# malaire/reed-solomon-16

Measured on AMD Instinct MI355X. Metric: encode+decode GiB/s (device-resident, 1024B shards); % of HBM roofline, higher is better.
Workload: dtype u16; 1 GPU; 32768:32768 x 1024 B encode + 100%-loss decode per GPU (BASELINE configs[3]); original_count=32768, recovery_count=32768, parallelism=independent stripes x 1 (weak, no collective), column_slices=1, decode_issue=serial: rs16_decode_device after the encode

## Files before the change

include/rs16.h:

```cpp
#ifndef RS16_H
#define RS16_H

#include <stddef.h>
#include <stdint.h>

#ifdef __cplusplus
extern "C" {
#endif

typedef enum rs16_error_code {
    RS16_OK = 0,
    RS16_DIFFERENT_SHARD_SIZE = 1,
    RS16_DUPLICATE_ORIGINAL_SHARD_INDEX = 2,
    RS16_DUPLICATE_RECOVERY_SHARD_INDEX = 3,
    RS16_INVALID_ORIGINAL_SHARD_INDEX = 4,
    RS16_INVALID_RECOVERY_SHARD_INDEX = 5,
    RS16_INVALID_SHARD_SIZE = 6,
    RS16_NOT_ENOUGH_SHARDS = 7,
    RS16_TOO_FEW_ORIGINAL_SHARDS = 8,
    RS16_TOO_MANY_ORIGINAL_SHARDS = 9,
    RS16_UNSUPPORTED_SHARD_COUNT = 10,
    RS16_DEVICE_ERROR = 100,
    RS16_INVALID_ARGUMENT = 101
} rs16_error_code;
// ... 174 lines not shown
int rs16_engine_set_stamps(rs16_engine* eng, void* d_buf, int prog, rs16_error* err);
const char* rs16_prog_name(int prog);

enum {
    RS16_DIAG_FORCE_VOFF64 = 1,
    RS16_DIAG_EVAL_TWO_KERNEL = 2,
    RS16_DIAG_EVAL_FULL = 4,
    RS16_DIAG_NO_COLUMN = 8,
    RS16_DIAG_FORCE_COLUMN = 16,
    RS16_DIAG_TILE_LAST = 32,
    RS16_DIAG_NO_TILE_LAST = 64,
    RS16_DIAG_FD_LDS = 128,
    RS16_DIAG_COL_RADIX4 = 256,
    RS16_DIAG_NO_IDENTITY = 512,
    RS16_DIAG_NO_MID_DIRECT = 1024,
    RS16_DIAG_WIDE_TWIDDLES = 2048
};
int rs16_engine_set_diagnostics(rs16_engine* eng, int flags);
int rs16_set_diagnostics(int flags);

void rs16_host_mul(const void* in, void* out, size_t bytes, uint16_t log_m);
void rs16_host_mul_narrow(const void* in, void* out, size_t bytes, uint16_t log_m);
uint32_t rs16_host_twiddle(uint32_t index, uint32_t* log_m, uint32_t* table20);
int rs16_host_twiddle_narrow(uint32_t index);
uint64_t rs16_host_fast_div_check(uint32_t divisor, uint32_t n0, uint32_t count, uint32_t step);
typedef struct rs16_pass_consts {
    uint32_t voff32, full_lanes, nslab;
    uint32_t quads, threads, load_shb, store_shb, reg_bits, row_sets;
    uint64_t rs_in, rs_seg, rs_out;
} rs16_pass_consts;
int rs16_host_pass_consts(int prog, int T, uint32_t lo, uint64_t s_in, uint64_t s_out, uint64_t s_seg, uint64_t s_rest,
                          uint32_t qrow, uint32_t chunk, uint32_t row_base_in, uint32_t in_rows_mask, int diag,
                          rs16_pass_consts* out);
int rs16_host_pass_consts_many(int prog, int T, uint32_t lo, size_t n, const uint64_t* s_in, const uint64_t* s_out,
                               const uint64_t* s_seg, const uint64_t* s_rest, const uint32_t* qrow, uint32_t chunk,
                               uint32_t row_base_in, uint32_t in_rows_mask, int diag, rs16_pass_consts* out);
int rs16_host_update_consts(uint32_t rows, uint64_t shard_bytes, uint32_t n, uint32_t* quads_per_lane,
                            uint32_t* nslab, uint32_t* rows_per_wave, uint64_t* blocks);

const char* rs16_version(void);

#ifdef __cplusplus
}
#endif
#endif
```

reed-solomon-16_amd/csrc/rs16_api.cpp:

```cpp
#include <atomic>
#include <rccl/rccl.h>

#include <algorithm>
#include <cstdio>
#include <cstring>
#include <new>
#include <vector>

#include "rs16_engine.hpp"
#include "rs16_pass_common.hpp"

using namespace rs16;

extern "C" size_t rs16_error_message(const rs16_error* e, char* buf, size_t len) {
    char tmp[256];
    unsigned long long a = e->v0, b = e->v1, c = e->v2;
    switch (e->code) {
    case RS16_OK: snprintf(tmp, sizeof tmp, "ok"); break;
    case RS16_DIFFERENT_SHARD_SIZE:
        snprintf(tmp, sizeof tmp, "different shard size: expected %llu bytes, got %llu bytes", a, b);
        break;
    case RS16_DUPLICATE_ORIGINAL_SHARD_INDEX: snprintf(tmp, sizeof tmp, "duplicate original shard index: %llu", a); break;
    case RS16_DUPLICATE_RECOVERY_SHARD_INDEX: snprintf(tmp, sizeof tmp, "duplicate recovery shard index: %llu", a); break;
    case RS16_INVALID_ORIGINAL_SHARD_INDEX:
// ... 68 lines not shown
    const HostTables& t = host_tables();
    if (index >= GF_MODULUS) return ~0u;
    if (log_m) *log_m = t.skew[index];
    if (table20) memcpy(table20, &t.skew_tab[(size_t)index * TAB_DWORDS], 20 * sizeof(uint32_t));
    return t.skew[index] == GF_MODULUS ? 0u : t.exp[t.skew[index]];
}
extern "C" int rs16_host_twiddle_narrow(uint32_t index) { return twiddle_narrow(index) ? 1 : 0; }
extern "C" uint64_t rs16_host_fast_div_check(uint32_t divisor, uint32_t n0, uint32_t count, uint32_t step) {
    const FastDiv f = fast_div_of(divisor);
    uint64_t bad = 0;
    for (uint64_t i = 0, n = n0; i < count && n < ((uint64_t)1 << 32); i++, n += step)
        bad += fast_div((uint32_t)n, f.mul, f.one) != (uint32_t)n / divisor;
    return bad;
}

extern "C" int rs16_host_pass_consts_many(int prog, int T, uint32_t lo, size_t n, const uint64_t* s_in,
                                          const uint64_t* s_out, const uint64_t* s_seg, const uint64_t* s_rest,
                                          const uint32_t* qrow, uint32_t chunk, uint32_t row_base_in,
                                          uint32_t in_rows_mask, int diag, rs16_pass_consts* out) {
    if (prog < 0 || prog >= NUM_PROGS || T < 0 || T > 8 || !out) return 0;
    const PassKernel& k = pass_kernel_of(prog, T);
    if (!k.fn) return 0;
    PassArgs a{};
    a.lo = lo, a.chunk = chunk, a.row_base_in = row_base_in, a.in_rows_mask = in_rows_mask;
    a.diag = (uint32_t)diag;
    for (size_t i = 0; i < n; i++) {
        a.S_in = s_in[i], a.S_out = s_out[i], a.S_seg = s_seg[i], a.S_rest = s_rest[i], a.qrow = qrow[i];
        const PassConsts c = pass_launch_consts(k, T, a);
        rs16_pass_consts& o = out[i];
        o.voff32 = c.voff32, o.full_lanes = c.full_lanes, o.nslab = c.nslab;
        o.quads = (uint32_t)k.quads, o.threads = (uint32_t)k.threads;
        o.load_shb = (uint32_t)k.load_shb, o.store_shb = (uint32_t)k.store_shb;
        o.reg_bits = (uint32_t)k.reg_bits, o.row_sets = k.quads >= 64 ? 1u : 64u / (uint32_t)k.quads;
        o.rs_in = c.rs_in, o.rs_seg = c.rs_seg, o.rs_out = c.rs_out;
    }
    return 1;
}
extern "C" int rs16_host_pass_consts(int prog, int T, uint32_t lo, uint64_t s_in, uint64_t s_out, uint64_t s_seg,
                                     uint64_t s_rest, uint32_t qrow, uint32_t chunk, uint32_t row_base_in,
                                     uint32_t in_rows_mask, int diag, rs16_pass_consts* out) {
    return rs16_host_pass_consts_many(prog, T, lo, 1, &s_in, &s_out, &s_seg, &s_rest, &qrow, chunk, row_base_in,
                                      in_rows_mask, diag, out);
}
extern "C" int rs16_host_update_consts(uint32_t rows, uint64_t shard_bytes, uint32_t n, uint32_t* quads_per_lane,
                                       uint32_t* nslab, uint32_t* rows_per_wave, uint64_t* blocks) {
    if (shard_bytes == 0 || (shard_bytes & 63) != 0 || shard_bytes / 8 > 0xFFFFFFFFu) return 0;
    UpdateArgs a{};
    a.S = shard_bytes, a.qrow = (uint32_t)(shard_bytes / 8), a.rows = rows;
    uint64_t nb;
    if (!update_launch_consts(a, n, &nb)) return 0;
    if (quads_per_lane) *quads_per_lane = a.quads_per_lane;
// ... 47 lines not shown
        for (uint32_t i = 0; i < g.a_count; i++) a += f[i] != 0;
        for (uint32_t i = 0; i < g.b_count; i++) b += f[GF_ORDER + i] != 0;
    } else {
        const size_t chunks = ((size_t)g.n + 63) / 64;
        std::vector<uint32_t> c(2 * chunks);
        RS16_HIP(hipMemcpy(c.data(), e->ev_main.rcount.p, c.size() * 4, hipMemcpyDeviceToHost));
        for (size_t i = 0; i < chunks; i++) a += c[2 * i], b += c[2 * i + 1];
    }
    const uint64_t want_o = g.high ? g.b_recv : g.a_recv, want_r = g.high ? g.a_recv : g.b_recv;
    const uint64_t got_o = g.high ? b : a, got_r = g.high ? a : b;
    if (got_o != want_o || got_r != want_r) return set_error(err, RS16_INVALID_ARGUMENT, got_o, got_r);
    return set_error(err, RS16_OK);
}
static constexpr int DIAG_ALL = DIAG_FORCE_VOFF64 | DIAG_EVAL_TWO_KERNEL | DIAG_EVAL_FULL | DIAG_NO_COLUMN |
                                DIAG_FORCE_COLUMN | DIAG_TILE_LAST | DIAG_NO_TILE_LAST | DIAG_FD_LDS |
                                DIAG_COL_RADIX4 | DIAG_NO_IDENTITY | DIAG_NO_MID_DIRECT | DIAG_WIDE_TWIDDLES;
extern "C" int rs16_engine_set_diagnostics(rs16_engine* e, int flags) {
    const int old = e->diag;
    e->diag = flags & DIAG_ALL;
    return old;
}
static std::atomic<int> g_default_diag{0};
extern "C" int rs16_set_diagnostics(int flags) { return g_default_diag.exchange(flags & DIAG_ALL); }
extern "C" int rs16_prog_count(void) { return NUM_PROF; }
extern "C" const char* rs16_prog_name(int prog) {
    static const char* names[] = {"GEN_FFT",   "GEN_IFFT",   "ENC_FIRST",     "ENC_MID",
                                  "ENC_LAST",  "ENC_SINGLE", "DEC_FIRST",     "DEC_MID",
                                  "DEC_LAST",  "DEC_SINGLE", "DEC_HALF_LAST", "DEC_HALF_SINGLE",
                                  "DEC_HALF_FIRST", "DEC_HALF_MID", "EVAL_POLY", "COL_ENC", "COL_DEC",
                                  "DEC_MID_DIRECT", "DEC_TILE_LAST"};
    static_assert(sizeof names / sizeof names[0] == NUM_PROF, "profiling names");
// ... 1546 lines not shown
```

reed-solomon-16_amd/csrc/rs16_diag.hpp:

```cpp
#pragma once
#include <hip/hip_runtime.h>
#include <stdint.h>

#ifndef RS16_STAMPS
#define RS16_STAMPS 0
#endif

#if RS16_STAMPS
namespace rs16 {
template <class Args>
__device__ __forceinline__ void diag_stamp(const Args& a, int i) {
    if (a.stamps && threadIdx.x == 0) {
        uint64_t* p = a.stamps + blockIdx.x * 16;
        p[i] = __builtin_amdgcn_s_memtime();
        if (i == 0) {
            p[14] = __builtin_amdgcn_s_memrealtime();
            p[12] = __builtin_amdgcn_s_getreg((31 << 11) | 4);
            p[13] = __builtin_amdgcn_s_getreg((31 << 11) | 20);
        }
        if (i == 11) p[15] = __builtin_amdgcn_s_memrealtime();
    }
}
}
#define RS16_STAMP(args, i) ::rs16::diag_stamp((args), (i))
// ... 16 lines not shown
```

reed-solomon-16_amd/csrc/rs16_internal.hpp:

```cpp
#pragma once
#include <hip/hip_runtime.h>
#include <stddef.h>
#include <stdint.h>

#include <vector>

#include "rs16_gf.hpp"

namespace rs16 {

struct HostTables {
    std::vector<uint16_t> exp, log, skew, log_walsh;
    std::vector<uint32_t> skew_entry;
    std::vector<uint32_t> mul_tab;
    std::vector<uint32_t> skew_tab;
    std::vector<uint32_t> col_img;
    std::vector<uint32_t> col_v;
    std::vector<uint32_t> col_k;
};
std::vector<uint32_t> mid_matrix_entries(const HostTables& t, int L);

constexpr uint32_t COL_LMIN = 6, COL_LMAX = 10;
constexpr uint32_t COL_LGEN = 11;
constexpr uint32_t COL_LCHUNK = 8;
// ... 155 lines not shown
hipError_t launch_col_multi(const ColArgs& a, bool high, hipStream_t s);

enum DiagFlags : int {
    DIAG_FORCE_VOFF64 = 1,
    DIAG_EVAL_TWO_KERNEL = 2,
    DIAG_EVAL_FULL = 4,
    DIAG_NO_COLUMN = 8,
    DIAG_FORCE_COLUMN = 16,
    DIAG_TILE_LAST = 32,
    DIAG_NO_TILE_LAST = 64,
    DIAG_FD_LDS = 128,
    DIAG_COL_RADIX4 = 256,
    DIAG_NO_IDENTITY = 512,
    DIAG_NO_MID_DIRECT = 1024,
    DIAG_WIDE_TWIDDLES = 2048,
};

constexpr size_t RS16_ZERO_BYTES = 65536;

hipError_t launch_pass(int prog, int T, const PassArgs& a, uint32_t num_tiles, hipStream_t s);
hipError_t launch_tile_last(const PassArgs& a, uint32_t num_tiles, hipStream_t s);
constexpr uint32_t MID_DIRECT_MAX = 4;
constexpr uint32_t TILE_LAST_MAX = 16;
hipError_t launch_mid_direct(const PassArgs& a, const uint32_t* mtab, uint32_t hi, uint32_t ns, hipStream_t s);

hipError_t launch_mul(uint8_t* x, size_t bytes, uint32_t entry, const uint32_t* mul_tab, hipStream_t s);
hipError_t launch_xor(uint8_t* x, const uint8_t* y, size_t bytes, hipStream_t s);
hipError_t launch_xor_chunks(uint8_t* w, size_t chunk_bytes, uint32_t nch, hipStream_t s);
hipError_t launch_copy_chunks(uint8_t* w, size_t chunk_bytes, uint32_t nch, hipStream_t s);
hipError_t launch_formal_derivative(uint8_t* out, const uint8_t* in, size_t shard_count, size_t S, hipStream_t s);
// ... 43 lines not shown
```

reed-solomon-16_amd/csrc/rs16_pass.hpp:

```cpp
#pragma once
#include "rs16_pass_common.hpp"
#include "rs16_fwht.hpp"
#include "rs16_diag.hpp"

namespace rs16 {

enum LoadMode { LD_PLAIN = 0, LD_GATHER_ENC, LD_GATHER_DEC, LD_DEC_LAST };
enum StoreMode { ST_PLAIN = 0, ST_RECOVERY, ST_RESTORE };

template <int P> struct ProgTraits;
#define RS16_PROG(P, LD, I, F, FF, ST)          \
    template <> struct ProgTraits<P> {         \
        static constexpr int LOAD = LD;        \
        static constexpr bool IFFT = I;        \
        static constexpr bool FD = F;          \
        static constexpr bool FFT = FF;        \
        static constexpr int STORE = ST;       \
        static constexpr bool ST_NT = !(I && FF);                                           \
    };
RS16_PROG(GEN_FFT, LD_PLAIN, false, false, true, ST_PLAIN)
RS16_PROG(GEN_IFFT, LD_PLAIN, true, false, false, ST_PLAIN)
RS16_PROG(ENC_FIRST, LD_GATHER_ENC, true, false, false, ST_PLAIN)
RS16_PROG(ENC_MID, LD_PLAIN, true, false, true, ST_PLAIN)
RS16_PROG(ENC_LAST, LD_PLAIN, false, false, true, ST_RECOVERY)
// ... 172 lines not shown
    }
    asm volatile("; full-item rows requested");
    return true;
}
enum RowsMode { ROWS_DIRECT = 0, ROWS_ZERO, ROWS_GENERAL };
template <int P, int T>
__device__ __forceinline__ uint32_t wave_rows_mode(const PassArgs& a, const Thr& c) {
    constexpr bool START_B = !ProgTraits<P>::IFFT;
    constexpr bool GATHER = ProgTraits<P>::LOAD == LD_GATHER_ENC;
    const WaveRows<T, START_B> wr(c, a);
    const bool below = !GATHER || wave_rows_end<T, START_B>(wr) <= a.a_count;
    const bool above = GATHER && wr.base >= a.a_count;
    const bool direct = (a.voff32 != 0) & (a.in_rows_mask == 0) & below;
    return direct ? ROWS_DIRECT : (above ? ROWS_ZERO : ROWS_GENERAL);
}
template <int P, int T> struct FastStore {
    static constexpr bool END_B = !ProgTraits<P>::FFT && T > 4;
    const PassArgs& a;
    const Thr& cs;
    bool on;
    uint64_t p;
    __device__ __forceinline__ FastStore(const PassArgs& a_, const Thr& cs_) : a(a_), cs(cs_), on(false), p(0) {
        if constexpr (FastRows<P, T>::STORE) {
            const WaveRows<T, END_B> wr(cs, a);
            on = a.full_lanes &&
                 (ProgTraits<P>::STORE != ST_RECOVERY || wave_rows_end<T, END_B>(wr) <= a.out_rows);
            p = (uint64_t)a.out + (uint64_t)wr.base * a.S_out;
        }
    }
    __device__ __forceinline__ void row(int m, uint32_t L, uint32_t H) const {
// ... 77 lines not shown
    }
};

template <int T> struct RevealEntry {
    const PassArgs& a;
    const Thr& c;
    const uint32_t* el;
    __device__ __forceinline__ uint32_t operator()(int k) const {
        const uint32_t r = row_rel<T>(c, a, (uint32_t)k) + a.row_base_out;
        return row_lost_original(a, r) ? GF_MODULUS - (el ? el[k] : a.elog[r]) : ZERO_ENTRY;
    }
};

struct NoFin {
    template <class X> __device__ __forceinline__ void operator()(const X&, const X&, int) const {}
};

template <int T, bool LB, int KB0, int KB1, bool FFT> struct LayerSeq {
    static constexpr int SH = LB ? Geo<T>::SHB : 0;
    static constexpr int NR = Geo<T>::NR;
    static constexpr bool DF = FFT && !LB && KB0 == 0 && KB1 == Geo<T>::R && NR >= 8;
    static constexpr int df_at(int g) {
        int skb[16] = {}, sgi[16] = {};
        int sp = 0, n = 0;
        skb[sp] = KB1 - 1, sgi[sp] = 0, sp++;
        while (sp > 0) {
            sp--;
            const int kb = skb[sp], gi = sgi[sp];
            if (n++ == g) return kb * 16 + gi;
            if (kb > 0) {
// ... 43 lines not shown
            asm volatile("" : "+v"(L[i]), "+v"(L[i + 1]), "+v"(L[i + 2]), "+v"(L[i + 3]), "+v"(H[i]), "+v"(H[i + 1]),
                         "+v"(H[i + 2]), "+v"(H[i + 3]));
    } else {
#pragma unroll
        for (int i = 0; i < NR; i++) asm volatile("" : "+v"(L[i]), "+v"(H[i]));
    }
}

enum { PR_NONE = 0, PR_OUT, PR_ZERO };
template <int NV> struct NarrowVar {
    static constexpr int NONE = 99;
    static constexpr int IFFT_FROM = NV == 0 ? NONE : (NV == 2 ? 1 : 0);
    static constexpr int FFT_FROM = NV == 0 ? NONE : (NV == 3 ? 1 : 0);
};

template <int P, int T, int NK, bool LB, int KB0, int KB1, bool FFT, bool IN_TAB2, int PRUNE, int G, class FIN = NoFin>
struct GroupLoop {
    static __device__ __forceinline__ void run(uint32_t (&L)[Geo<T>::NR], uint32_t (&H)[Geo<T>::NR], const Thr& c,
                                               const PassArgs& a, const uint4* tab1, const uint4* tab2,
                                               const uint32_t (&cur)[20], uint32_t zmask, const FIN& fin = FIN()) {
        using S = LayerSeq<T, LB, KB0, KB1, FFT>;
        constexpr int s = S::step_of(G), gi = S::index_of(G);
        constexpr int kb = S::kb_of(s);
        constexpr int rb = kb - S::SH;
        constexpr bool more = G + 1 < S::total();
        constexpr bool NARROW = kb >= NK;
        uint32_t nxt[20];
        if constexpr (more)
            load_table_lds(nxt, group_table<T, LB, KB0, KB1, FFT, G + 1, IN_TAB2>(c, tab1, tab2));
        __builtin_amdgcn_sched_barrier(0);
        bool need = true;
        if constexpr (PRUNE == PR_OUT)
            need = ((uint32_t)gi << (kb + 1)) < a.need_hi && ((uint32_t)(gi + 1) << (kb + 1)) > a.need_lo;
        if constexpr (PRUNE == PR_ZERO) {
            static_assert(LB && kb >= 4, "zero pruning works on 16-row blocks of layout B");
            constexpr int nb = 1 << (kb - 3);
            constexpr uint32_t all = (uint32_t)((1ull << nb) - 1);
            need = ((zmask >> (gi * nb)) & all) != all;
        }
        bool mul = true;
        if constexpr (LB && gi == 0 && ProgTraits<P>::IFFT && ProgTraits<P>::FFT) {
            const uint32_t idx = (c.b_high << (a.lo + T)) + (1u << (a.lo + kb)) + (FFT ? a.skew_fft : a.skew_ifft) - 1;
            mul = (idx & (idx + 1)) != 0;
        }
        if (need && mul) {
#pragma unroll
            for (int j = 0; j < (1 << rb); j++) {
                const int m = (gi << (rb + 1)) + j, m2 = m + (1 << rb);
                if (FFT) {
                    mul_xor_t<NARROW>(L[m], H[m], L[m2], H[m2], cur);
                    L[m2] ^= L[m];
                    H[m2] ^= H[m];
                } else {
                    L[m2] ^= L[m];
                    H[m2] ^= H[m];
                    mul_xor_t<NARROW>(L[m], H[m], L[m2], H[m2], cur);
                }
            }
        } else if (need) {
#pragma unroll
            for (int j = 0; j < (1 << rb); j++) {
                const int m = (gi << (rb + 1)) + j, m2 = m + (1 << rb);
                L[m2] ^= L[m];
                H[m2] ^= H[m];
            }
        }
#pragma unroll
        for (int j = 0; j < (1 << rb); j++) {
            const int m = (gi << (rb + 1)) + j, m2 = m + (1 << rb);
            asm volatile("" : "+v"(L[m]), "+v"(H[m]), "+v"(L[m2]), "+v"(H[m2]));
        }
        __builtin_amdgcn_sched_barrier(0);
        if constexpr (S::DF && kb == 0) fin(L, H, gi << 1);
        if constexpr (more)
            GroupLoop<P, T, NK, LB, KB0, KB1, FFT, IN_TAB2, PRUNE, G + 1, FIN>::run(L, H, c, a, tab1, tab2, nxt, zmask,
                                                                                     fin);
    }
};

__device__ __forceinline__ const uint4* lds_vgpr(const uint4* p) {
    uint32_t v = (uint32_t)(uintptr_t)(const __attribute__((address_space(3))) uint4*)p;
    asm volatile("" : "+v"(v));
    return (const uint4*)(const __attribute__((address_space(3))) uint4*)(uintptr_t)v;
}

template <int P, int T, int NK, bool LB, int KB0, int KB1, bool FFT, bool IN_TAB2, int PRUNE = PR_NONE,
          class FIN = NoFin>
__device__ __forceinline__ void layers(uint32_t (&L)[Geo<T>::NR], uint32_t (&H)[Geo<T>::NR], const Thr& c,
                                       const PassArgs& a, const uint4* tab1, const uint4* tab2,
                                       uint32_t zmask = 0, const FIN& fin = FIN()) {
    if constexpr (KB1 > KB0) {
        if constexpr (LB) {
            if constexpr (IN_TAB2) tab2 = lds_vgpr(tab2);
            else tab1 = lds_vgpr(tab1);
        }
        uint32_t t0[20];
        load_table_lds(t0, group_table<T, LB, KB0, KB1, FFT, 0, IN_TAB2>(c, tab1, tab2));
        GroupLoop<P, T, NK, LB, KB0, KB1, FFT, IN_TAB2, PRUNE, 0, FIN>::run(L, H, c, a, tab1, tab2, t0, zmask, fin);
    }
}

template <int T, int QL> struct Img {
    static constexpr int PLANE = (1 << T) * QL;
    static __device__ __forceinline__ uint32_t* at(uint2* lds, const Thr& c, uint32_t k) {
        return (uint32_t*)lds + k * QL + c.ql;
    }
};

template <int NQR> __device__ __forceinline__ bool my_round(const Thr& c, int r) {
    return NQR == 1 || c.round == (uint32_t)r;
}

template <int T, int QL, bool LB>
// ... 573 lines not shown
    const FastStore<P, T> fs;
    __device__ __forceinline__ void operator()(const uint32_t (&L)[Geo<T>::NR], const uint32_t (&H)[Geo<T>::NR]) const {
        if (fs.on) {
#pragma unroll
            for (int m = 0; m < Geo<T>::NR; m += 2) fs.row(m, L[m], H[m]);
            return;
        }
#pragma unroll
        for (int m = 0; m < Geo<T>::NR; m += 2) {
            if (a.voff32) store_row<P, T, true>(a, cs, L[m], H[m], m, nullptr, nullptr);
            else store_row<P, T, false>(a, cs, L[m], H[m], m, nullptr, nullptr);
        }
    }
};

template <int P, int T, int NV>
__device__ __forceinline__ void process_item(const PassArgs& a, const Thr& c, uint32_t tile, ItemRegs<P, T>& d,
                                             uint8_t* smem) {
    using PT = ProgTraits<P>;
    constexpr int NKI = NarrowVar<NV>::IFFT_FROM, NKF = NarrowVar<NV>::FFT_FROM;
    static_assert(NV == 0 || (PT::IFFT && PT::FFT && T > 4), "narrow variants: two-direction passes only");
    using SM = Smem<P, T>;
    using G = Geo<T>;
    constexpr int NR = G::NR;
    constexpr int R = G::R;
    constexpr int NQR = Rnd<P, T>::NQR;
    constexpr bool TWO = SM::TWO;
    constexpr bool ZERO_SKIP = P == DEC_MID && T > 4 && G::R == 4;
    constexpr bool EARLY = LayerSeq<T, false, 0, R, true>::DF && P != DEC_MID && PT::STORE != ST_RESTORE && PT::FFT &&
                           T > 4;
    constexpr bool EARLY_B = PT::IFFT && !PT::FFT && PT::STORE == ST_PLAIN && T > 4 && G::R == 4;
    uint2* lds = (uint2*)smem;
    const uint4* tab1 = (const uint4*)(smem + SM::TAB1_OFF);
// ... 32 lines not shown
            const uint32_t yl = L[m], yh = H[m];
            L[m] = H[m] = 0;
            mul_xor(L[m], H[m], yl, yh, tt);
        }
    }
    if constexpr (PT::LOAD == LD_DEC_LAST) {
        if (!d.ztile) tile_fd<T, NQR, START_B>(L, H, d.zl, d.zh, c, lds);
    }

    [[maybe_unused]] Stager<T, (SM::SHARED ? G::TSPLIT : 0)> s3s;
    bool in_b = START_B;
    if constexpr (PT::IFFT) {
        bool skip_a = false;
        if constexpr (ZERO_SKIP) skip_a = __all(d.zrow == (1u << NR) - 1);
        if constexpr (WaveStaged<P, T>::value) RS16_STAMP_ROWS(a, 6, L, H, 0, 1);
        if (!skip_a) layers<P, T, NKI, false, 0, R, false, false>(L, H, c, a, tab1, tab2);
        RS16_STAMP(a, 3);
        prio<1>();
        if constexpr (T > 4) {
            constexpr bool LS2 = SM::RESTAGE && !SM::SHARED;
            Stager<T, (LS2 ? G::TSPLIT : 0)> s3;
            if constexpr (LS2) s3.issue(a.skew_tab, TwiddleEntry<T>{a, c, 0, a.skew_fft});
            if constexpr (SM::SHARED) __syncthreads();
            exchange<T, NQR, false>(
                L, H, c, lds,
                [&]() {
                    if constexpr (LS2) s3.commit((uint4*)(smem + SM::TAB1_OFF));
                },
                [&]() {
                    if constexpr (SPLIT_FD) {
                        if (fd_few) {
// ... 21 lines not shown
        prio<2>();
    }
    if constexpr (PT::FD) {
        if constexpr (SPLIT_FD) {
            if (fd_few) fd_regs<T>(L, H);
            else tile_fd<T, NQR, true>(L, H, L, H, c, lds);
        } else {
            if (in_b) tile_fd<T, NQR, true>(L, H, L, H, c, lds);
            else tile_fd<T, NQR, false>(L, H, L, H, c, lds);
        }
        RS16_STAMP(a, 6);
    }
    if constexpr (PT::FFT) {
        if constexpr (T > 4) {
            if constexpr (WaveStaged<P, T>::value && !PT::IFFT) RS16_STAMP_ROWS(a, 6, L, H, 0, NR / 2);
            layers<P, T, NKF, true, R, (T > 4 ? T : R), true, TWO, (P == DEC_MID ? PR_OUT : PR_NONE)>(L, H, c, a, tab1,
                                                                                                  tab2);
            if constexpr (SPLIT_FD) {
                if (fd_few) {
#pragma unroll
                    for (int m = 0; m < NR; m++) {
#pragma unroll
                        for (int i = 0; i < FD_ND; i++)
                            if ((uint32_t)m == fd_m0 + i) L[m] ^= dl[i], H[m] ^= dh[i];
                    }
                }
            }
            RS16_STAMP(a, 7);
            prio<3>();
            RevealStage<P, (LateReveal<P, T>::value ? T : 0)> rs;
            if constexpr (LateReveal<P, T>::value) {
                const uint32_t* el = nullptr;
// ... 148 lines not shown
            lost_range(a, r0, r1);
            const bool any = r0 < r1;
            a.need_lo = max(a.need_lo, any ? r0 >> a.lo : 0u);
            a.need_hi = min(a.need_hi, any ? ((r1 - 1) >> a.lo) + 1 : 0u);
        }
    }
    RS16_STAMP(a, 1);
    prio<0>();
    st.template finish<EARLY>(a, c, smem);
    rcn.count();
    RS16_STAMP(a, 2);
    process_item<P, T, NV>(a, c, tile, cur, smem);
    rcn.store(a, c);
}

template <int P, int T, int NV = 0> PassKernel pass_entry() {
    using PT = ProgTraits<P>;
    return {pass_kernel<P, T, NV>, Smem<P, T>::BYTES, Geo<T>::THREADS, Geo<T>::Q,
            !PT::IFFT ? Geo<T>::SHB : 0, (!PT::FFT && T > 4) ? Geo<T>::SHB : 0, Geo<T>::R};
}
template <int P> PassKernel pass_row(int T) {
    static const PassKernel row[9] = {pass_entry<P, 0>(), pass_entry<P, 1>(), pass_entry<P, 2>(),
                                      pass_entry<P, 3>(), pass_entry<P, 4>(), pass_entry<P, 5>(),
                                      pass_entry<P, 6>(), pass_entry<P, 7>(), pass_entry<P, 8>()};
    return row[T];
}
template <int P, int NV> PassKernel narrow_row(int T) {
    static const PassKernel row[4] = {pass_entry<P, 5, NV>(), pass_entry<P, 6, NV>(), pass_entry<P, 7, NV>(),
                                      pass_entry<P, 8, NV>()};
    return T >= 5 ? row[T - 5] : PassKernel{};
}

}
```

reed-solomon-16_amd/csrc/rs16_pass_common.hpp:

```cpp
#pragma once
#include "rs16_internal.hpp"

namespace rs16 {

typedef void (*PassFn)(PassArgs);
struct PassKernel {
    PassFn fn;
    int lds;
    int threads;
    int quads;
    int load_shb, store_shb;
    int reg_bits;
};
struct PassConsts {
    uint32_t nslab, voff32, full_lanes;
    uint64_t rs_in, rs_seg, rs_out;
};
PassConsts pass_launch_consts(const PassKernel& k, int T, const PassArgs& a);
const PassKernel& pass_kernel_of(int prog, int T);
constexpr int NARROW_VARIANTS = 4;
PassKernel pass_kernels_enc(int prog, int T, int nv);
PassKernel pass_kernels_dec(int prog, int T, int nv);

#if defined(__HIPCC__) || defined(__HIP__)
typedef const __attribute__((address_space(4))) uint32_t* cu32p;

__device__ __forceinline__ uint32_t uni(uint32_t v) { return __builtin_amdgcn_readfirstlane(v); }

__host__ __device__ constexpr int vmcnt_wait(int n) { return (n & 15) | ((n >> 4) << 14) | (7 << 4) | (15 << 8); }

__device__ __forceinline__ void load_table_lds(uint32_t (&t)[20], const uint4* p) {
// ... 59 lines not shown
```

reed-solomon-16_amd/csrc/rs16_pass_launch.hip:

```cpp
#include <algorithm>

#include "rs16_pass_common.hpp"

namespace rs16 {

struct KernelTable {
    PassKernel k[NUM_PROGS][9][NARROW_VARIANTS];
    KernelTable() {
        for (int prog = 0; prog < NUM_PROGS; prog++)
            for (int T = 0; T <= 8; T++)
                for (int nv = 0; nv < NARROW_VARIANTS; nv++) {
                    const PassKernel e = pass_kernels_enc(prog, T, nv);
                    k[prog][T][nv] = e.fn ? e : pass_kernels_dec(prog, T, nv);
                }
    }
};
static const PassKernel& find_kernel(int prog, int T, int nv) {
    static const KernelTable table;
    return table.k[prog][T][nv];
}

static const PassKernel& pick_kernel(int prog, int T, int ni, int nf) {
    for (int nv = 1; nv < NARROW_VARIANTS; nv++) {
        const int vi = nv == 2 ? 1 : 0, vf = nv == 3 ? 1 : 0;
// ... 10 lines not shown
    PassConsts c;
    c.nslab = (a.qrow + k.quads - 1) / k.quads;
    {
        const uint64_t hws = k.quads >= 64 ? 1 : 64 / k.quads;
        const uint64_t smax = std::max(std::max(a.S_in, a.S_out), std::max(a.S_seg, a.S_rest));
        const uint64_t span = (uint64_t)1 << (T + a.lo);
        const bool fits = (hws - 1) * ((uint64_t)16 << a.lo) * smax + 8 * (uint64_t)a.qrow <= ((uint64_t)1 << 32);
        const bool aligned = a.chunk % span == 0 && a.row_base_in % span == 0;
        c.voff32 = fits && aligned && !(a.diag & DIAG_FORCE_VOFF64) ? 1u : 0u;
    }
    c.rs_in = a.S_in << (a.lo + k.load_shb);
    c.rs_seg = a.S_seg << (a.lo + k.load_shb);
    c.rs_out = a.S_out << (a.lo + k.store_shb);
    const bool full = c.voff32 && a.qrow % k.quads == 0 && a.in_rows_mask == 0 && c.rs_out < ((uint64_t)1 << 28);
    c.full_lanes = full ? 1u : 0u;
    return c;
}

hipError_t launch_pass(int prog, int T, const PassArgs& args, uint32_t num_tiles, hipStream_t s) {
    if (prog < 0 || prog >= NUM_PROGS || T < 0 || T > 8) return hipErrorInvalidValue;
    if (num_tiles == 0 || args.qrow == 0) return hipSuccess;
    PassArgs a = args;
    int ni = T, nf = T;
    if (!(a.diag & DIAG_WIDE_TWIDDLES)) {
        const uint32_t bh_max = (a.tile_base + (a.stripe_tiles ? a.stripe_tiles : num_tiles) - 1) >> a.lo;
        ni = first_narrow_layer(a.lo, T, a.skew_ifft, bh_max);
        nf = first_narrow_layer(a.lo, T, a.skew_fft, bh_max);
    }
    const PassKernel& k = pick_kernel(prog, T, ni, nf);
    const PassConsts pc = pass_launch_consts(k, T, a);
    a.nslab = pc.nslab;
    a.ntiles = num_tiles;
    const uint32_t nwg = num_tiles * a.nslab;
    if (a.need_hi == 0) a.need_hi = 1u << T;
    a.voff32 = pc.voff32;
    a.fd_lds = (a.diag & DIAG_FD_LDS) ? 1u : 0u;
    a.rs_in = pc.rs_in, a.rs_seg = pc.rs_seg, a.rs_out = pc.rs_out;
    a.full_lanes = pc.full_lanes;
    const FastDiv dn = fast_div_of(a.nslab), ds = fast_div_of(a.stripe_tiles);
    a.nslab_mul = dn.mul, a.nslab_one = dn.one;
    a.stripe_mul = ds.mul, a.stripe_one = ds.one;
    const size_t lds = (size_t)k.lds;
    if (lds > 65536) {
        hipError_t e = hipFuncSetAttribute((const void*)k.fn, hipFuncAttributeMaxDynamicSharedMemorySize, (int)lds);
        if (e != hipSuccess) return e;
    }
    dim3 grid(nwg), block(k.threads);
    hipLaunchKernelGGL(k.fn, grid, block, lds, s, a);
    return hipGetLastError();
}

}
```

reed-solomon-16_amd/rs16/__init__.py:

```python
from __future__ import annotations

import atexit
import ctypes as C
import weakref
from typing import Iterable, Iterator, Optional, Tuple

import numpy as np

from ._lib import RS16Error, lib

__all__ = [
    "Error", "Engine", "default_engine", "ReedSolomonEncoder", "ReedSolomonDecoder", "RateEncoder",
    "RateDecoder", "EncoderResult", "DecoderResult", "encode", "decode", "encode_device", "decode_device",
    "supports", "validate", "use_high_rate", "encode_device_batch", "decode_device_batch", "encoder_work_count", "decoder_work_count",
    "RATE_DEFAULT", "RATE_HIGH", "RATE_LOW", "GF_ORDER", "GF_MODULUS", "set_diagnostics",
    "DIAG_FORCE_VOFF64", "DIAG_EVAL_TWO_KERNEL", "DIAG_EVAL_FULL", "DIAG_NO_COLUMN", "DIAG_FORCE_COLUMN",
    "DIAG_TILE_LAST", "DIAG_NO_TILE_LAST", "DIAG_FD_LDS", "DIAG_COL_RADIX4", "DIAG_NO_IDENTITY", "DIAG_NO_MID_DIRECT", "DIAG_WIDE_TWIDDLES", "encode_host", "decode_host",
    "encode_host_batch", "decode_host_batch", "decode_prepare", "decode_device_prepared",
    "UpdatePlan", "update_recovery_device", "UPDATE_MAX_SHARDS",
    "encode_host_multi", "decode_host_multi", "Comm", "column_slice", "scatter_columns", "gather_columns",
]

GF_ORDER = 65536
GF_MODULUS = 65535
DIAG_FORCE_VOFF64, DIAG_EVAL_TWO_KERNEL, DIAG_EVAL_FULL, DIAG_NO_COLUMN, DIAG_FORCE_COLUMN = 1, 2, 4, 8, 16
DIAG_TILE_LAST, DIAG_NO_TILE_LAST, DIAG_FD_LDS, DIAG_COL_RADIX4, DIAG_NO_IDENTITY = 32, 64, 128, 256, 512
DIAG_NO_MID_DIRECT = 1024
DIAG_WIDE_TWIDDLES = 2048
_diag_default = 0


def set_diagnostics(flags: int, engine: Optional["Engine"] = None) -> int:
    global _diag_default
    if engine is not None:
        return engine.set_diagnostics(flags)
    old, _diag_default = _diag_default, flags
    for e in list(_live_engines):
        if getattr(e, "h", None):
            e.set_diagnostics(flags)
    return old
RATE_DEFAULT, RATE_HIGH, RATE_LOW = 0, 1, 2
_RATES = {"default": 0, "high": 1, "low": 2, 0: 0, 1: 1, 2: 2}

# ... 797 lines not shown
```

reed-solomon-16_amd/rs16/_lib.py:

```python
from __future__ import annotations

import ctypes as C
import os
from pathlib import Path

PKG_ROOT = Path(__file__).resolve().parents[1]
LIB_PATH = Path(os.environ.get("RS16_LIB", PKG_ROOT / "build" / "librs16.so"))


class RS16Error(C.Structure):
    _fields_ = [("code", C.c_int32), ("v0", C.c_uint64), ("v1", C.c_uint64), ("v2", C.c_uint64)]


class PassConsts(C.Structure):
    _fields_ = [(n, C.c_uint32) for n in ("voff32", "full_lanes", "nslab", "quads", "threads", "load_shb",
                                          "store_shb", "reg_bits", "row_sets")] + \
               [(n, C.c_uint64) for n in ("rs_in", "rs_seg", "rs_out")]


_sz, _p, _i, _e = C.c_size_t, C.c_void_p, C.c_int, C.POINTER(RS16Error)
_u32, _u64 = C.c_uint32, C.c_uint64

SIGNATURES = {
    "rs16_error_message": (_sz, [_e, C.c_char_p, _sz]),
    "rs16_version": (C.c_char_p, []),
    "rs16_host_mul": (None, [_p, _p, _sz, C.c_uint16]),
    "rs16_host_mul_narrow": (None, [_p, _p, _sz, C.c_uint16]),
    "rs16_host_twiddle": (C.c_uint32, [C.c_uint32, C.POINTER(C.c_uint32), C.POINTER(C.c_uint32)]),
    "rs16_host_twiddle_narrow": (C.c_int, [C.c_uint32]),
    "rs16_host_fast_div_check": (C.c_uint64, [C.c_uint32, C.c_uint32, C.c_uint32, C.c_uint32]),
    "rs16_host_pass_consts": (_i, [_i, _i, _u32, _u64, _u64, _u64, _u64, _u32, _u32, _u32, _u32, _i,
                                   C.POINTER(PassConsts)]),
    "rs16_host_pass_consts_many": (_i, [_i, _i, _u32, _sz, _p, _p, _p, _p, _p, _u32, _u32, _u32, _i, _p]),
    "rs16_host_update_consts": (_i, [_u32, _u64, _u32, C.POINTER(_u32), C.POINTER(_u32), C.POINTER(_u32),
                                     C.POINTER(_u64)]),
    "rs16_engine_set_profiling": (_i, [_p, _i, _e]),
    "rs16_engine_profile_read": (_i, [_p, _i, C.POINTER(C.c_double), C.POINTER(C.c_uint64), _e]),
    "rs16_engine_profile_reset": (None, [_p]),
    "rs16_prog_count": (_i, []),
    "rs16_engine_set_diagnostics": (_i, [_p, _i]),
    "rs16_prog_name": (C.c_char_p, [_i]),
    "rs16_engine_set_stamps": (_i, [_p, _p, _i, _e]),
    "rs16_engine_set_slices": (_i, [_p, _i, _e]),
    "rs16_engine_new": (_p, [_i, _e]),
    "rs16_engine_new_ex": (_p, [_i, _i, _e]),
    "rs16_set_diagnostics": (_i, [_i]),
    "rs16_engine_free": (None, [_p]),
# ... 111 lines not shown
```

Baseline: 1012 GiB/s.

## Stream late row pairs into registers during first butterfly layer in wave-staged passes

Adds a variant pass kernel for wave-staged programs that loads only the first D row pairs up front and fetches the remaining pairs from global memory inside the first layer of the IFFT/FFT butterfly loop, interleaved with compute. The aim is to overlap global-load latency with the GF multiply-xor work instead of waiting for all rows before computing. The host selects this kernel when strides fit in 32-bit offsets, no row mask is set and gather row counts align, with a diagnostic flag to disable it. The cost is extra scheduling barriers and register pressure, and the zero-skip shortcut is bypassed on this path.

```diff
diff --git a/include/rs16.h b/include/rs16.h
--- a/include/rs16.h
+++ b/include/rs16.h
@@ -212,7 +212,8 @@
     RS16_DIAG_COL_RADIX4 = 256,
     RS16_DIAG_NO_IDENTITY = 512,
     RS16_DIAG_NO_MID_DIRECT = 1024,
-    RS16_DIAG_WIDE_TWIDDLES = 2048
+    RS16_DIAG_WIDE_TWIDDLES = 2048,
+    RS16_DIAG_NO_LATE_ROWS = 4096
 };
 int rs16_engine_set_diagnostics(rs16_engine* eng, int flags);
 int rs16_set_diagnostics(int flags);
@@ -226,6 +227,7 @@
     uint32_t voff32, full_lanes, nslab;
     uint32_t quads, threads, load_shb, store_shb, reg_bits, row_sets;
     uint64_t rs_in, rs_seg, rs_out;
+    uint32_t late_rows;
 } rs16_pass_consts;
 int rs16_host_pass_consts(int prog, int T, uint32_t lo, uint64_t s_in, uint64_t s_out, uint64_t s_seg, uint64_t s_rest,
                           uint32_t qrow, uint32_t chunk, uint32_t row_base_in, uint32_t in_rows_mask, int diag,
@@ -233,6 +235,9 @@
 int rs16_host_pass_consts_many(int prog, int T, uint32_t lo, size_t n, const uint64_t* s_in, const uint64_t* s_out,
                                const uint64_t* s_seg, const uint64_t* s_rest, const uint32_t* qrow, uint32_t chunk,
                                uint32_t row_base_in, uint32_t in_rows_mask, int diag, rs16_pass_consts* out);
+int rs16_host_pass_consts_rows(int prog, int T, uint32_t lo, uint64_t s_in, uint64_t s_out, uint64_t s_seg,
+                               uint64_t s_rest, uint32_t qrow, uint32_t chunk, uint32_t row_base_in,
+                               uint32_t in_rows_mask, uint32_t a_count, int diag, rs16_pass_consts* out);
 int rs16_host_update_consts(uint32_t rows, uint64_t shard_bytes, uint32_t n, uint32_t* quads_per_lane,
                             uint32_t* nslab, uint32_t* rows_per_wave, uint64_t* blocks);
 
diff --git a/reed-solomon-16_amd/csrc/rs16_api.cpp b/reed-solomon-16_amd/csrc/rs16_api.cpp
--- a/reed-solomon-16_amd/csrc/rs16_api.cpp
+++ b/reed-solomon-16_amd/csrc/rs16_api.cpp
@@ -106,16 +106,17 @@
     return bad;
 }
 
-extern "C" int rs16_host_pass_consts_many(int prog, int T, uint32_t lo, size_t n, const uint64_t* s_in,
-                                          const uint64_t* s_out, const uint64_t* s_seg, const uint64_t* s_rest,
-                                          const uint32_t* qrow, uint32_t chunk, uint32_t row_base_in,
-                                          uint32_t in_rows_mask, int diag, rs16_pass_consts* out) {
+static int host_pass_consts(int prog, int T, uint32_t lo, size_t n, const uint64_t* s_in, const uint64_t* s_out,
+                            const uint64_t* s_seg, const uint64_t* s_rest, const uint32_t* qrow, uint32_t chunk,
+                            uint32_t row_base_in, uint32_t in_rows_mask, uint32_t a_count, int diag,
+                            rs16_pass_consts* out) {
     if (prog < 0 || prog >= NUM_PROGS || T < 0 || T > 8 || !out) return 0;
     const PassKernel& k = pass_kernel_of(prog, T);
     if (!k.fn) return 0;
     PassArgs a{};
     a.lo = lo, a.chunk = chunk, a.row_base_in = row_base_in, a.in_rows_mask = in_rows_mask;
     a.diag = (uint32_t)diag;
+    a.a_count = a_count;
     for (size_t i = 0; i < n; i++) {
         a.S_in = s_in[i], a.S_out = s_out[i], a.S_seg = s_seg[i], a.S_rest = s_rest[i], a.qrow = qrow[i];
         const PassConsts c = pass_launch_consts(k, T, a);
@@ -125,8 +126,22 @@
         o.load_shb = (uint32_t)k.load_shb, o.store_shb = (uint32_t)k.store_shb;
         o.reg_bits = (uint32_t)k.reg_bits, o.row_sets = k.quads >= 64 ? 1u : 64u / (uint32_t)k.quads;
         o.rs_in = c.rs_in, o.rs_seg = c.rs_seg, o.rs_out = c.rs_out;
+        o.late_rows = c.late_rows;
     }
     return 1;
+}
+extern "C" int rs16_host_pass_consts_many(int prog, int T, uint32_t lo, size_t n, const uint64_t* s_in,
+                                          const uint64_t* s_out, const uint64_t* s_seg, const uint64_t* s_rest,
+                                          const uint32_t* qrow, uint32_t chunk, uint32_t row_base_in,
+                                          uint32_t in_rows_mask, int diag, rs16_pass_consts* out) {
+    return host_pass_consts(prog, T, lo, n, s_in, s_out, s_seg, s_rest, qrow, chunk, row_base_in, in_rows_mask, 0, diag,
+                            out);
+}
+extern "C" int rs16_host_pass_consts_rows(int prog, int T, uint32_t lo, uint64_t s_in, uint64_t s_out, uint64_t s_seg,
+                                          uint64_t s_rest, uint32_t qrow, uint32_t chunk, uint32_t row_base_in,
+                                          uint32_t in_rows_mask, uint32_t a_count, int diag, rs16_pass_consts* out) {
+    return host_pass_consts(prog, T, lo, 1, &s_in, &s_out, &s_seg, &s_rest, &qrow, chunk, row_base_in, in_rows_mask,
+                            a_count, diag, out);
 }
 extern "C" int rs16_host_pass_consts(int prog, int T, uint32_t lo, uint64_t s_in, uint64_t s_out, uint64_t s_seg,
                                      uint64_t s_rest, uint32_t qrow, uint32_t chunk, uint32_t row_base_in,
@@ -204,7 +219,8 @@
 }
 static constexpr int DIAG_ALL = DIAG_FORCE_VOFF64 | DIAG_EVAL_TWO_KERNEL | DIAG_EVAL_FULL | DIAG_NO_COLUMN |
                                 DIAG_FORCE_COLUMN | DIAG_TILE_LAST | DIAG_NO_TILE_LAST | DIAG_FD_LDS |
-                                DIAG_COL_RADIX4 | DIAG_NO_IDENTITY | DIAG_NO_MID_DIRECT | DIAG_WIDE_TWIDDLES;
+                                DIAG_COL_RADIX4 | DIAG_NO_IDENTITY | DIAG_NO_MID_DIRECT | DIAG_WIDE_TWIDDLES |
+                                DIAG_NO_LATE_ROWS;
 extern "C" int rs16_engine_set_diagnostics(rs16_engine* e, int flags) {
     const int old = e->diag;
     e->diag = flags & DIAG_ALL;
diff --git a/reed-solomon-16_amd/csrc/rs16_diag.hpp b/reed-solomon-16_amd/csrc/rs16_diag.hpp
--- a/reed-solomon-16_amd/csrc/rs16_diag.hpp
+++ b/reed-solomon-16_amd/csrc/rs16_diag.hpp
@@ -4,6 +4,10 @@
 
 #ifndef RS16_STAMPS
 #define RS16_STAMPS 0
+#endif
+
+#ifndef RS16_LATE_DEPTH
+#define RS16_LATE_DEPTH 0
 #endif
 
 #if RS16_STAMPS
diff --git a/reed-solomon-16_amd/csrc/rs16_internal.hpp b/reed-solomon-16_amd/csrc/rs16_internal.hpp
--- a/reed-solomon-16_amd/csrc/rs16_internal.hpp
+++ b/reed-solomon-16_amd/csrc/rs16_internal.hpp
@@ -193,6 +193,7 @@
     DIAG_NO_IDENTITY = 512,
     DIAG_NO_MID_DIRECT = 1024,
     DIAG_WIDE_TWIDDLES = 2048,
+    DIAG_NO_LATE_ROWS = 4096,
 };
 
 constexpr size_t RS16_ZERO_BYTES = 65536;
diff --git a/reed-solomon-16_amd/csrc/rs16_pass.hpp b/reed-solomon-16_amd/csrc/rs16_pass.hpp
--- a/reed-solomon-16_amd/csrc/rs16_pass.hpp
+++ b/reed-solomon-16_amd/csrc/rs16_pass.hpp
@@ -1,4 +1,6 @@
 #pragma once
+#include <type_traits>
+
 #include "rs16_pass_common.hpp"
 #include "rs16_fwht.hpp"
 #include "rs16_diag.hpp"
@@ -210,6 +212,55 @@
     const bool direct = (a.voff32 != 0) & (a.in_rows_mask == 0) & below;
     return direct ? ROWS_DIRECT : (above ? ROWS_ZERO : ROWS_GENERAL);
 }
+template <int P> struct LateDepth {
+    static constexpr int SHIPPED = 8;
+    static constexpr int value = RS16_LATE_DEPTH > 0 ? RS16_LATE_DEPTH : SHIPPED;
+};
+template <int P, int T> struct LateRows {
+    using G = Geo<T>;
+    static constexpr bool START_B = !ProgTraits<P>::IFFT;
+    static constexpr bool GATHER = ProgTraits<P>::LOAD == LD_GATHER_ENC;
+    static constexpr int RB = START_B ? G::R - 1 : 0;
+    static constexpr int NP = G::NR / 2;
+    static constexpr int D = LateDepth<P>::value < NP ? LateDepth<P>::value : NP;
+    static_assert(D >= 1 && G::R == 4, "late rows: 16-row sets");
+    uint64_t p;
+    uint32_t rs, voff;
+    __device__ __forceinline__ LateRows(const PassArgs& a, const Thr& c) {
+        const WaveRows<T, START_B> wr(c, a);
+        const bool rows = !GATHER || wr.base < a.a_count;
+        const uint64_t S = GATHER ? a.S_seg : a.S_in;
+        const uint32_t offL = !c.active ? ((c.offL >> 6) - (c.qt >> 3)) * 64 : c.offL;
+        rs = rows ? (uint32_t)(GATHER ? a.rs_seg : a.rs_in) : 0u;
+        voff = rows ? lane_rows<T, START_B>(c, a) * (uint32_t)S + offL : (c.offL & 0x7FFFu);
+        p = rows ? (uint64_t)(GATHER ? a.seg_a : a.in) + (uint64_t)wr.base * S : (uint64_t)a.zero;
+    }
+    __device__ __forceinline__ void pair(uint32_t (&L)[G::NR], uint32_t (&H)[G::NR], int q) const {
+        const int m = ((q >> RB) << (RB + 1)) + (q & ((1 << RB) - 1));
+        uint32_t v = voff;
+        asm volatile("" : "+v"(v));
+#pragma unroll
+        for (int i = 0; i < 2; i++) {
+            const int mi = m + (i << RB);
+            const gu32* g = (const gu32*)(sgpr_ptr((const uint8_t*)(p + (uint32_t)mi * rs)) + v);
+            L[mi] = g[0];
+            H[mi] = g[8];
+        }
+    }
+    __device__ __forceinline__ void prologue(uint32_t (&L)[G::NR], uint32_t (&H)[G::NR]) const {
+#pragma unroll
+        for (int q = 0; q < D; q++) pair(L, H, q);
+        asm volatile("; late rows: prologue requested");
+    }
+    __device__ __forceinline__ void operator()(uint32_t (&L)[G::NR], uint32_t (&H)[G::NR], int q) const {
+        if (q + D < NP) {
+            __builtin_amdgcn_sched_barrier(0);
+            pair(L, H, q + D);
+            __builtin_amdgcn_sched_barrier(0);
+        }
+    }
+};
+
 template <int P, int T> struct FastStore {
     static constexpr bool END_B = !ProgTraits<P>::FFT && T > 4;
     const PassArgs& a;
@@ -317,6 +368,9 @@
 
 struct NoFin {
     template <class X> __device__ __forceinline__ void operator()(const X&, const X&, int) const {}
+};
+struct NoPre {
+    template <class X> __device__ __forceinline__ void operator()(X&, X&, int) const {}
 };
 
 template <int T, bool LB, int KB0, int KB1, bool FFT> struct LayerSeq {
@@ -390,11 +444,13 @@
     static constexpr int FFT_FROM = NV == 0 ? NONE : (NV == 3 ? 1 : 0);
 };
 
-template <int P, int T, int NK, bool LB, int KB0, int KB1, bool FFT, bool IN_TAB2, int PRUNE, int G, class FIN = NoFin>
+template <int P, int T, int NK, bool LB, int KB0, int KB1, bool FFT, bool IN_TAB2, int PRUNE, int G, class FIN = NoFin,
+          class PRE = NoPre>
 struct GroupLoop {
     static __device__ __forceinline__ void run(uint32_t (&L)[Geo<T>::NR], uint32_t (&H)[Geo<T>::NR], const Thr& c,
                                                const PassArgs& a, const uint4* tab1, const uint4* tab2,
-                                               const uint32_t (&cur)[20], uint32_t zmask, const FIN& fin = FIN()) {
+                                               const uint32_t (&cur)[20], uint32_t zmask, const FIN& fin = FIN(),
+                                               const PRE& pre = PRE()) {
         using S = LayerSeq<T, LB, KB0, KB1, FFT>;
         constexpr int s = S::step_of(G), gi = S::index_of(G);
         constexpr int kb = S::kb_of(s);
@@ -423,6 +479,7 @@
 #pragma unroll
             for (int j = 0; j < (1 << rb); j++) {
                 const int m = (gi << (rb + 1)) + j, m2 = m + (1 << rb);
+                if constexpr (!std::is_same<PRE, NoPre>::value && s == 0) pre(L, H, (gi << rb) + j);
                 if (FFT) {
                     mul_xor_t<NARROW>(L[m], H[m], L[m2], H[m2], cur);
                     L[m2] ^= L[m];
@@ -449,8 +506,8 @@
         __builtin_amdgcn_sched_barrier(0);
         if constexpr (S::DF && kb == 0) fin(L, H, gi << 1);
         if constexpr (more)
-            GroupLoop<P, T, NK, LB, KB0, KB1, FFT, IN_TAB2, PRUNE, G + 1, FIN>::run(L, H, c, a, tab1, tab2, nxt, zmask,
-                                                                                     fin);
+            GroupLoop<P, T, NK, LB, KB0, KB1, FFT, IN_TAB2, PRUNE, G + 1, FIN, PRE>::run(L, H, c, a, tab1, tab2, nxt,
+                                                                                          zmask, fin, pre);
     }
 };
 
@@ -461,10 +518,10 @@
 }
 
 template <int P, int T, int NK, bool LB, int KB0, int KB1, bool FFT, bool IN_TAB2, int PRUNE = PR_NONE,
-          class FIN = NoFin>
+          class FIN = NoFin, class PRE = NoPre>
 __device__ __forceinline__ void layers(uint32_t (&L)[Geo<T>::NR], uint32_t (&H)[Geo<T>::NR], const Thr& c,
                                        const PassArgs& a, const uint4* tab1, const uint4* tab2,
-                                       uint32_t zmask = 0, const FIN& fin = FIN()) {
+                                       uint32_t zmask = 0, const FIN& fin = FIN(), const PRE& pre = PRE()) {
     if constexpr (KB1 > KB0) {
         if constexpr (LB) {
             if constexpr (IN_TAB2) tab2 = lds_vgpr(tab2);
@@ -472,7 +529,8 @@
         }
         uint32_t t0[20];
         load_table_lds(t0, group_table<T, LB, KB0, KB1, FFT, 0, IN_TAB2>(c, tab1, tab2));
-        GroupLoop<P, T, NK, LB, KB0, KB1, FFT, IN_TAB2, PRUNE, 0, FIN>::run(L, H, c, a, tab1, tab2, t0, zmask, fin);
+        GroupLoop<P, T, NK, LB, KB0, KB1, FFT, IN_TAB2, PRUNE, 0, FIN, PRE>::run(L, H, c, a, tab1, tab2, t0, zmask, fin,
+                                                                                 pre);
     }
 }
 
@@ -1076,9 +1134,9 @@
     }
 };
 
-template <int P, int T, int NV>
+template <int P, int T, int NV, class PRE = NoPre>
 __device__ __forceinline__ void process_item(const PassArgs& a, const Thr& c, uint32_t tile, ItemRegs<P, T>& d,
-                                             uint8_t* smem) {
+                                             uint8_t* smem, const PRE& pre = PRE()) {
     using PT = ProgTraits<P>;
     constexpr int NKI = NarrowVar<NV>::IFFT_FROM, NKF = NarrowVar<NV>::FFT_FROM;
     static_assert(NV == 0 || (PT::IFFT && PT::FFT && T > 4), "narrow variants: two-direction passes only");
@@ -1141,7 +1199,9 @@
         bool skip_a = false;
         if constexpr (ZERO_SKIP) skip_a = __all(d.zrow == (1u << NR) - 1);
         if constexpr (WaveStaged<P, T>::value) RS16_STAMP_ROWS(a, 6, L, H, 0, 1);
-        if (!skip_a) layers<P, T, NKI, false, 0, R, false, false>(L, H, c, a, tab1, tab2);
+        if constexpr (!std::is_same<PRE, NoPre>::value)
+            layers<P, T, NKI, false, 0, R, false, false, PR_NONE, NoFin, PRE>(L, H, c, a, tab1, tab2, 0, NoFin(), pre);
+        else if (!skip_a) layers<P, T, NKI, false, 0, R, false, false>(L, H, c, a, tab1, tab2);
         RS16_STAMP(a, 3);
         prio<1>();
         if constexpr (T > 4) {
@@ -1193,8 +1253,11 @@
     if constexpr (PT::FFT) {
         if constexpr (T > 4) {
             if constexpr (WaveStaged<P, T>::value && !PT::IFFT) RS16_STAMP_ROWS(a, 6, L, H, 0, NR / 2);
-            layers<P, T, NKF, true, R, (T > 4 ? T : R), true, TWO, (P == DEC_MID ? PR_OUT : PR_NONE)>(L, H, c, a, tab1,
-                                                                                                  tab2);
+            if constexpr (!std::is_same<PRE, NoPre>::value && !PT::IFFT)
+                layers<P, T, NKF, true, R, T, true, TWO, PR_NONE, NoFin, PRE>(L, H, c, a, tab1, tab2, 0, NoFin(), pre);
+            else
+                layers<P, T, NKF, true, R, (T > 4 ? T : R), true, TWO, (P == DEC_MID ? PR_OUT : PR_NONE)>(L, H, c, a, tab1,
+                                                                                                      tab2);
             if constexpr (SPLIT_FD) {
                 if (fd_few) {
 #pragma unroll
@@ -1373,10 +1436,66 @@
     rcn.store(a, c);
 }
 
+template <int P, int T, int NV = 0>
+__global__ void __launch_bounds__(Geo<T>::THREADS, 4) pass_kernel_late(PassArgs a) {
+    using G = Geo<T>;
+    static_assert(WaveStaged<P, T>::value, "late rows: the wave-staged passes");
+    extern __shared__ __attribute__((aligned(16))) uint8_t smem[];
+    const uint32_t item = blockIdx.x;
+
+    Thr c;
+    c.lane = threadIdx.x & 63;
+    c.w = uni(threadIdx.x >> 6);
+    c.qt = c.lane % G::Q;
+    c.s = c.w * G::HWS + c.lane / G::Q;
+    c.ql = c.qt % Rnd<P, T>::QL;
+    c.round = c.qt / Rnd<P, T>::QL;
+
+    uint32_t tile, slab;
+    set_item(c, a, item, G::Q, tile, slab);
+
+    bool first_stripe = true;
+    if (a.stripe_tiles) {
+        const uint32_t st = uni(fast_div(tile, a.stripe_mul, a.stripe_one));
+        first_stripe = st == 0;
+        tile -= st * a.stripe_tiles;
+        stripe_displace(a, st);
+    }
+    tile += a.tile_base;
+    c.b_low = tile & ((1u << a.lo) - 1);
+    c.b_high = tile >> a.lo;
+    RcvCount<P, T> rcn;
+    rcn.issue(a, c, slab == 0 && first_stripe);
+    RS16_STAMP(a, 0);
+    const uint32_t slot = (__builtin_amdgcn_s_getreg((31 << 11) | 4) >> 16) & 15u;
+    if (slot == 0) __builtin_amdgcn_s_setprio(3);
+    else if (slot == 1) __builtin_amdgcn_s_setprio(2);
+    else if (slot == 2) __builtin_amdgcn_s_setprio(1);
+    TileStage<P, T> st;
+    st.issue(a, c);
+    ItemRegs<P, T> cur;
+    cur.zrow = cur.zmask = 0;
+    cur.ztile = false;
+    const LateRows<P, T> rq(a, c);
+    rq.prologue(cur.L, cur.H);
+    RS16_STAMP(a, 1);
+    prio<0>();
+    st.template finish<false>(a, c, smem);
+    rcn.count();
+    RS16_STAMP(a, 2);
+    process_item<P, T, NV, LateRows<P, T>>(a, c, tile, cur, smem, rq);
+    rcn.store(a, c);
+}
+
+template <int P, int T, int NV> PassFn late_entry() {
+    if constexpr (WaveStaged<P, T>::value) return pass_kernel_late<P, T, NV>;
+    else return nullptr;
+}
 template <int P, int T, int NV = 0> PassKernel pass_entry() {
     using PT = ProgTraits<P>;
     return {pass_kernel<P, T, NV>, Smem<P, T>::BYTES, Geo<T>::THREADS, Geo<T>::Q,
-            !PT::IFFT ? Geo<T>::SHB : 0, (!PT::FFT && T > 4) ? Geo<T>::SHB : 0, Geo<T>::R};
+            !PT::IFFT ? Geo<T>::SHB : 0, (!PT::FFT && T > 4) ? Geo<T>::SHB : 0, Geo<T>::R,
+            late_entry<P, T, NV>(), PT::LOAD == LD_GATHER_ENC ? 1 : 0};
 }
 template <int P> PassKernel pass_row(int T) {
     static const PassKernel row[9] = {pass_entry<P, 0>(), pass_entry<P, 1>(), pass_entry<P, 2>(),
diff --git a/reed-solomon-16_amd/csrc/rs16_pass_common.hpp b/reed-solomon-16_amd/csrc/rs16_pass_common.hpp
--- a/reed-solomon-16_amd/csrc/rs16_pass_common.hpp
+++ b/reed-solomon-16_amd/csrc/rs16_pass_common.hpp
@@ -11,10 +11,13 @@
     int quads;
     int load_shb, store_shb;
     int reg_bits;
+    PassFn late;
+    int gather;
 };
 struct PassConsts {
     uint32_t nslab, voff32, full_lanes;
     uint64_t rs_in, rs_seg, rs_out;
+    uint32_t late_rows;
 };
 PassConsts pass_launch_consts(const PassKernel& k, int T, const PassArgs& a);
 const PassKernel& pass_kernel_of(int prog, int T);
diff --git a/reed-solomon-16_amd/csrc/rs16_pass_launch.hip b/reed-solomon-16_amd/csrc/rs16_pass_launch.hip
--- a/reed-solomon-16_amd/csrc/rs16_pass_launch.hip
+++ b/reed-solomon-16_amd/csrc/rs16_pass_launch.hip
@@ -48,6 +48,15 @@
     c.rs_out = a.S_out << (a.lo + k.store_shb);
     const bool full = c.voff32 && a.qrow % k.quads == 0 && a.in_rows_mask == 0 && c.rs_out < ((uint64_t)1 << 28);
     c.full_lanes = full ? 1u : 0u;
+    {
+        const uint64_t hws = k.quads >= 64 ? 1 : 64 / k.quads;
+        const uint64_t wave_span = (hws << k.reg_bits) << a.lo;
+        const bool whole = !k.gather || a.a_count % wave_span == 0;
+        const bool strides = c.rs_in < ((uint64_t)1 << 28) && c.rs_seg < ((uint64_t)1 << 28);
+        c.late_rows = k.late && c.voff32 && a.in_rows_mask == 0 && whole && strides && !(a.diag & DIAG_NO_LATE_ROWS)
+                          ? 1u
+                          : 0u;
+    }
     return c;
 }
 
@@ -75,12 +84,13 @@
     a.nslab_mul = dn.mul, a.nslab_one = dn.one;
     a.stripe_mul = ds.mul, a.stripe_one = ds.one;
     const size_t lds = (size_t)k.lds;
+    const PassFn fn = pc.late_rows ? k.late : k.fn;
     if (lds > 65536) {
-        hipError_t e = hipFuncSetAttribute((const void*)k.fn, hipFuncAttributeMaxDynamicSharedMemorySize, (int)lds);
+        hipError_t e = hipFuncSetAttribute((const void*)fn, hipFuncAttributeMaxDynamicSharedMemorySize, (int)lds);
         if (e != hipSuccess) return e;
     }
     dim3 grid(nwg), block(k.threads);
-    hipLaunchKernelGGL(k.fn, grid, block, lds, s, a);
+    hipLaunchKernelGGL(fn, grid, block, lds, s, a);
     return hipGetLastError();
 }
 
diff --git a/reed-solomon-16_amd/rs16/__init__.py b/reed-solomon-16_amd/rs16/__init__.py
--- a/reed-solomon-16_amd/rs16/__init__.py
+++ b/reed-solomon-16_amd/rs16/__init__.py
@@ -15,7 +15,7 @@
     "supports", "validate", "use_high_rate", "encode_device_batch", "decode_device_batch", "encoder_work_count", "decoder_work_count",
     "RATE_DEFAULT", "RATE_HIGH", "RATE_LOW", "GF_ORDER", "GF_MODULUS", "set_diagnostics",
     "DIAG_FORCE_VOFF64", "DIAG_EVAL_TWO_KERNEL", "DIAG_EVAL_FULL", "DIAG_NO_COLUMN", "DIAG_FORCE_COLUMN",
-    "DIAG_TILE_LAST", "DIAG_NO_TILE_LAST", "DIAG_FD_LDS", "DIAG_COL_RADIX4", "DIAG_NO_IDENTITY", "DIAG_NO_MID_DIRECT", "DIAG_WIDE_TWIDDLES", "encode_host", "decode_host",
+    "DIAG_TILE_LAST", "DIAG_NO_TILE_LAST", "DIAG_FD_LDS", "DIAG_COL_RADIX4", "DIAG_NO_IDENTITY", "DIAG_NO_MID_DIRECT", "DIAG_WIDE_TWIDDLES", "DIAG_NO_LATE_ROWS", "encode_host", "decode_host",
     "encode_host_batch", "decode_host_batch", "decode_prepare", "decode_device_prepared",
     "UpdatePlan", "update_recovery_device", "UPDATE_MAX_SHARDS",
     "encode_host_multi", "decode_host_multi", "Comm", "column_slice", "scatter_columns", "gather_columns",
@@ -27,6 +27,7 @@
 DIAG_TILE_LAST, DIAG_NO_TILE_LAST, DIAG_FD_LDS, DIAG_COL_RADIX4, DIAG_NO_IDENTITY = 32, 64, 128, 256, 512
 DIAG_NO_MID_DIRECT = 1024
 DIAG_WIDE_TWIDDLES = 2048
+DIAG_NO_LATE_ROWS = 4096
 _diag_default = 0
 
 
diff --git a/reed-solomon-16_amd/rs16/_lib.py b/reed-solomon-16_amd/rs16/_lib.py
--- a/reed-solomon-16_amd/rs16/_lib.py
+++ b/reed-solomon-16_amd/rs16/_lib.py
@@ -15,7 +15,7 @@
 class PassConsts(C.Structure):
     _fields_ = [(n, C.c_uint32) for n in ("voff32", "full_lanes", "nslab", "quads", "threads", "load_shb",
                                           "store_shb", "reg_bits", "row_sets")] + \
-               [(n, C.c_uint64) for n in ("rs_in", "rs_seg", "rs_out")]
+               [(n, C.c_uint64) for n in ("rs_in", "rs_seg", "rs_out")] + [("late_rows", C.c_uint32)]
 
 
 _sz, _p, _i, _e = C.c_size_t, C.c_void_p, C.c_int, C.POINTER(RS16Error)
@@ -31,6 +31,8 @@
     "rs16_host_fast_div_check": (C.c_uint64, [C.c_uint32, C.c_uint32, C.c_uint32, C.c_uint32]),
     "rs16_host_pass_consts": (_i, [_i, _i, _u32, _u64, _u64, _u64, _u64, _u32, _u32, _u32, _u32, _i,
                                    C.POINTER(PassConsts)]),
+    "rs16_host_pass_consts_rows": (_i, [_i, _i, _u32, _u64, _u64, _u64, _u64, _u32, _u32, _u32, _u32, _u32, _i,
+                                        C.POINTER(PassConsts)]),
     "rs16_host_pass_consts_many": (_i, [_i, _i, _u32, _sz, _p, _p, _p, _p, _p, _u32, _u32, _u32, _i, _p]),
     "rs16_host_update_consts": (_i, [_u32, _u64, _u32, C.POINTER(_u32), C.POINTER(_u32), C.POINTER(_u32),
                                      C.POINTER(_u64)]),
```

Result: faster. 1050 GiB/s (median of 6 runs) (+3.7%).
